# haosulab/ActiveZero

Hardware: AMD Instinct MI355X
Metric: stereo pairs/sec (540x960, D=192) fwd+bwd (higher is better)
Workload: dtype f32; 1 GPU; configs[1]: PSMNet 540x960 (padded to 544 rows) D=192 fwd+bwd+Adam, supervised disparity loss, batch 4 per GPU; global_batch=4, height=540, width=960, maxdisp=192, parallelism=dp1

## Files before the change

### activezero_amd/csrc/az_conv3d_c1.hip

```cpp
#include "az_common.h"
#include "az_launch_math.h"

#define C1_TH 8
#define C1_TW 32
#define C1_VS 36
#define C1_GP 36
typedef float c1_f2 __attribute__((ext_vector_type(2)));
#define C1_FMA2(a, b, c) __builtin_elementwise_fma(a, b, c)


#define C1F_TH 8
#define C1F_TW 16
template <int CTRL>
__device__ __forceinline__ float c1_dpp_add(float v) {
    return v + __builtin_bit_cast(float, __builtin_amdgcn_update_dpp(0, __builtin_bit_cast(int, v), CTRL, 0xf, 0xf, true));
}
__global__ void __launch_bounds__(256)
c1_fwd_kernel(float *__restrict__ out, const float *__restrict__ in, const float *__restrict__ w,
              const float *__restrict__ addend, const float *__restrict__ in_scale,
              const float *__restrict__ in_shift, int D, int H, int W, int tiles_x, int dseg) {
    constexpr int SX = C1F_TW + 2, SY = C1F_TH + 2;
    __shared__ __attribute__((aligned(16))) float slab[SY * SX * C1_VS];
    const int tx0 = (blockIdx.x % tiles_x) * C1F_TW, ty0 = (blockIdx.x / tiles_x) * C1F_TH;
    const int d0 = blockIdx.y * dseg, d1 = min(d0 + dseg, D), b = blockIdx.z;
    const int cp = threadIdx.x & 15, grp = threadIdx.x >> 4;
    const int ly = grp >> 1, lx0 = (grp & 1) * 8;
    const int oh = ty0 + ly;
    c1_f2 wp[27];
#pragma unroll
    for (int t = 0; t < 27; ++t) wp[t] = c1_f2{w[(cp * 2 + 0) * 27 + t], w[(cp * 2 + 1) * 27 + t]};
    c1_f2 a_prev[8], a_cur[8], a_next[8];
#pragma unroll
    for (int j = 0; j < 8; ++j) { a_prev[j] = c1_f2{0.f, 0.f}; a_cur[j] = c1_f2{0.f, 0.f}; a_next[j] = c1_f2{0.f, 0.f}; }
    constexpr int NQ = SY * SX * 8, NLD = (NQ + 255) / 256;
    float4 pre[NLD];
    const bool affine = in_scale != nullptr;
    float4 isc = make_float4(1.f, 1.f, 1.f, 1.f), ish = make_float4(0.f, 0.f, 0.f, 0.f);
    if (affine) {
        isc = reinterpret_cast<const float4 *>(in_scale)[threadIdx.x & 7];
        ish = reinterpret_cast<const float4 *>(in_shift)[threadIdx.x & 7];
    }
    unsigned okbits = 0;
    auto issue = [&](int id) {
        okbits = 0;
#pragma unroll
        for (int it = 0; it < NLD; ++it) {
            const int q = threadIdx.x + 256 * it, v = q >> 3, part = q & 7;
            const int sy = v / SX, sx = v - sy * SX;
            const int ih = ty0 - 1 + sy, iw = tx0 - 1 + sx;
            pre[it] = make_float4(0.f, 0.f, 0.f, 0.f);
            if (q < NQ && id >= 0 && id < D && ih >= 0 && ih < H && iw >= 0 && iw < W) {
                pre[it] = *reinterpret_cast<const float4 *>(
                    in + ((((size_t)b * D + id) * H + ih) * W + iw) * 32 + part * 4);
                okbits |= 1u << it;
            }
        }
    };
    issue(d0 - 1);
    for (int id = d0 - 1; id <= d1; ++id) {
        if (id >= 0 && id < D) {
            __syncthreads();
#pragma unroll
            for (int it = 0; it < NLD; ++it) {
                const int q = threadIdx.x + 256 * it;
                float4 v = pre[it];
                if (affine && ((okbits >> it) & 1u)) {
                    v.x = az_relu(fmaf(v.x, isc.x, ish.x)); v.y = az_relu(fmaf(v.y, isc.y, ish.y));
                    v.z = az_relu(fmaf(v.z, isc.z, ish.z)); v.w = az_relu(fmaf(v.w, isc.w, ish.w));
                }
                if (q < NQ) *reinterpret_cast<float4 *>(&slab[(q >> 3) * C1_VS + (q & 7) * 4]) = v;
            }
            __syncthreads();
        }
        if (id < d1) issue(id + 1);
        if (id >= 0 && id < D) {
#pragma unroll
            for (int kh = 0; kh < 3; ++kh) {
                c1_f2 r[10];
                const float *row = &slab[((ly + kh) * SX + lx0) * C1_VS + cp * 2];
#pragma unroll
                for (int i = 0; i < 10; ++i) {
                    const float2 x = *reinterpret_cast<const float2 *>(row + i * C1_VS);
                    r[i] = c1_f2{x.x, x.y};
                }
#pragma unroll
                for (int kw = 0; kw < 3; ++kw)
#pragma unroll
                    for (int j = 0; j < 8; ++j) {
                        a_next[j] = C1_FMA2(r[j + kw], wp[kh * 3 + kw], a_next[j]);
                        a_cur[j] = C1_FMA2(r[j + kw], wp[9 + kh * 3 + kw], a_cur[j]);
                        a_prev[j] = C1_FMA2(r[j + kw], wp[18 + kh * 3 + kw], a_prev[j]);
                    }
            }
        }
        const int od = id - 1;
        if (od >= d0 && od < d1) {
            float mine = 0.f;
#pragma unroll
            for (int j = 0; j < 8; ++j) {
                float v = a_prev[j][0] + a_prev[j][1];
                v = c1_dpp_add<0xB1>(v);
                v = c1_dpp_add<0x4E>(v);
                v = c1_dpp_add<0x141>(v);
                v = c1_dpp_add<0x140>(v);
                mine = (cp == j) ? v : mine;
            }
            const int ow = tx0 + lx0 + cp;
            if (cp < 8 && oh < H && ow < W) {
                const size_t o = (((size_t)b * D + od) * H + oh) * W + ow;
                out[o] = addend ? mine + addend[o] : mine;
            }
        }
#pragma unroll
        for (int j = 0; j < 8; ++j) { a_prev[j] = a_cur[j]; a_cur[j] = a_next[j]; a_next[j] = c1_f2{0.f, 0.f}; }
    }
}

__device__ __forceinline__ void c1_load_gtile(float *gt, const float *__restrict__ gout, int b,
                                              int od, int ty0, int tx0, int D, int H, int W) {
    constexpr int SX = C1_TW + 2, SY = C1_TH + 2;
    for (int q = threadIdx.x; q < 3 * SY * SX; q += 256) {
        const int sx = q % SX;
        const int r = q / SX;
        const int sy = r % SY, sd = r / SY;
        const int gd = od - 1 + sd, gh = ty0 - 1 + sy, gw = tx0 - 1 + sx;
        gt[r * C1_GP + sx] = (gd >= 0 && gd < D && gh >= 0 && gh < H && gw >= 0 && gw < W)
                                 ? gout[(((size_t)b * D + gd) * H + gh) * W + gw] : 0.f;
    }
}
__device__ __forceinline__ void c1_row6(float (&r)[6], const float *gt, int pd, int sy, int lx0) {
    const float *row = static_cast<const float *>(__builtin_assume_aligned(gt + (pd * (C1_TH + 2) + sy) * C1_GP + lx0, 16));
    const float4 a = *reinterpret_cast<const float4 *>(row);
    const float2 c = *reinterpret_cast<const float2 *>(row + 4);
    r[0] = a.x; r[1] = a.y; r[2] = a.z; r[3] = a.w; r[4] = c.x; r[5] = c.y;
}

__global__ void __launch_bounds__(256)
c1_dgrad_kernel(float *__restrict__ gin, const float *__restrict__ gout,
                const float *__restrict__ w, int D, int H, int W, int tiles_x) {
    constexpr int SY = C1_TH + 2;
    __shared__ __attribute__((aligned(16))) float gt[3 * SY * C1_GP];
    const int tx0 = (blockIdx.x % tiles_x) * C1_TW, ty0 = (blockIdx.x / tiles_x) * C1_TH;
    const int od = blockIdx.y, b = blockIdx.z;
    c1_load_gtile(gt, gout, b, od, ty0, tx0, D, H, W);
    const int cp = threadIdx.x & 15, grp = threadIdx.x >> 4;
    c1_f2 wp[27];
#pragma unroll
    for (int t = 0; t < 27; ++t) wp[t] = c1_f2{w[(cp * 2 + 0) * 27 + t], w[(cp * 2 + 1) * 27 + t]};
    __syncthreads();
#pragma unroll 1
    for (int p = 0; p < C1_TH * C1_TW / 128; ++p) {
        const int gi = p * 16 + grp, ly = gi >> 2, lx0 = (gi & 3) * 8;
        const int oh = ty0 + ly;
        c1_f2 acc[8];
#pragma unroll
        for (int j = 0; j < 8; ++j) acc[j] = c1_f2{0.f, 0.f};
#pragma unroll
        for (int kd = 0; kd < 3; ++kd)
#pragma unroll
            for (int kh = 0; kh < 3; ++kh) {
                float r[12];
                {
                    const float *row = static_cast<const float *>(__builtin_assume_aligned(
                        gt + ((2 - kd) * SY + ly + 2 - kh) * C1_GP + lx0, 16));
                    const float4 a = *reinterpret_cast<const float4 *>(row);
                    const float4 c = *reinterpret_cast<const float4 *>(row + 4);
                    const float2 e = *reinterpret_cast<const float2 *>(row + 8);
                    r[0] = a.x; r[1] = a.y; r[2] = a.z; r[3] = a.w; r[4] = c.x; r[5] = c.y; r[6] = c.z; r[7] = c.w;
                    r[8] = e.x; r[9] = e.y;
                }
#pragma unroll
                for (int kw = 0; kw < 3; ++kw) {
                    const int t = (kd * 3 + kh) * 3 + kw;
#pragma unroll
                    for (int j = 0; j < 8; ++j) {
                        const c1_f2 g2 = {r[j + 2 - kw], r[j + 2 - kw]};
                        acc[j] = C1_FMA2(g2, wp[t], acc[j]);
                    }
                }
            }
#pragma unroll
        for (int j = 0; j < 8; ++j) asm volatile("" : "+v"(acc[j]));
        if (oh < H) {
            float *dst = gin + ((((size_t)b * D + od) * H + oh) * W + tx0 + lx0) * 32 + cp * 2;
#pragma unroll
            for (int j = 0; j < 8; ++j)
                if (tx0 + lx0 + j < W) *reinterpret_cast<float2 *>(dst + j * 32) = make_float2(acc[j][0], acc[j][1]);
        }
    }
}

__global__ void __launch_bounds__(256)
c1_wgrad_kernel(float *__restrict__ gw, const float *__restrict__ in,
                const float *__restrict__ gout, const float *__restrict__ in_scale,
                const float *__restrict__ in_shift, int D, int H, int W, int tiles_x, int tiles_y,
                long long ntiles) {
    constexpr int SY = C1_TH + 2;
    __shared__ __attribute__((aligned(16))) float gt[3 * SY * C1_GP];
    __shared__ float red[864];
    for (int q = threadIdx.x; q < 864; q += 256) red[q] = 0.f;
    const int quad = threadIdx.x & 7, grp = threadIdx.x >> 3;
    const bool affine = in_scale != nullptr;
    float4 isc = make_float4(1.f, 1.f, 1.f, 1.f), ish = make_float4(0.f, 0.f, 0.f, 0.f);
    if (affine) {
        isc = reinterpret_cast<const float4 *>(in_scale)[quad];
        ish = reinterpret_cast<const float4 *>(in_shift)[quad];
    }
    c1_f2 a01[27], a23[27];
#pragma unroll
    for (int t = 0; t < 27; ++t) { a01[t] = c1_f2{0.f, 0.f}; a23[t] = c1_f2{0.f, 0.f}; }
    for (long long item = blockIdx.x; item < ntiles; item += gridDim.x) {
        long long r = item;
        const int tx0 = (int)(r % tiles_x) * C1_TW; r /= tiles_x;
        const int ty0 = (int)(r % tiles_y) * C1_TH; r /= tiles_y;
        const int od = (int)(r % D);
        const int b = (int)(r / D);
        __syncthreads();
        c1_load_gtile(gt, gout, b, od, ty0, tx0, D, H, W);
        __syncthreads();
#pragma unroll 1
        for (int p = 0; p < C1_TH * C1_TW / 128; ++p) {
            const int gi = p * 32 + grp, ly = gi >> 3, lx0 = (gi & 7) * 4;
            const int ih = ty0 + ly;
            c1_f2 x01[4], x23[4];
            const float *src = in + ((((size_t)b * D + od) * H + ih) * W + tx0 + lx0) * 32 + quad * 4;
#pragma unroll
            for (int j = 0; j < 4; ++j) {
                float4 x = make_float4(0.f, 0.f, 0.f, 0.f);
                if (ih < H && tx0 + lx0 + j < W) {
                    x = *reinterpret_cast<const float4 *>(src + j * 32);
                    if (affine) {
                        x.x = az_relu(fmaf(x.x, isc.x, ish.x)); x.y = az_relu(fmaf(x.y, isc.y, ish.y));
                        x.z = az_relu(fmaf(x.z, isc.z, ish.z)); x.w = az_relu(fmaf(x.w, isc.w, ish.w));
                    }
                }
                x01[j] = c1_f2{x.x, x.y}; x23[j] = c1_f2{x.z, x.w};
            }
#pragma unroll
            for (int kd = 0; kd < 3; ++kd)
#pragma unroll
                for (int kh = 0; kh < 3; ++kh) {
                    float r[6];
                    c1_row6(r, gt, 2 - kd, ly + 2 - kh, lx0);
#pragma unroll
                    for (int kw = 0; kw < 3; ++kw) {
                        const int t = (kd * 3 + kh) * 3 + kw;
#pragma unroll
                        for (int j = 0; j < 4; ++j) {
                            const c1_f2 g2 = {r[j + 2 - kw], r[j + 2 - kw]};
                            a01[t] = C1_FMA2(g2, x01[j], a01[t]);
                            a23[t] = C1_FMA2(g2, x23[j], a23[t]);
                        }
                    }
                }
        }
    }
#pragma unroll
    for (int c = 0; c < 4; ++c)
#pragma unroll
        for (int t = 0; t < 27; ++t) {
            float v = (c < 2 ? a01[t] : a23[t])[c & 1];
            v += __shfl_xor(v, 8); v += __shfl_xor(v, 16); v += __shfl_xor(v, 32);
            if ((threadIdx.x & 63) < 8) atomicAdd(&red[(quad * 4 + c) * 27 + t], v);
        }
    __syncthreads();
    for (int q = threadIdx.x; q < 864; q += 256) atomicAdd(&gw[q], red[q]);
}

static int c1_check(int B, int D, int H, int W) {
    if (!(B > 0 && D > 0 && H > 0 && W > 0)) return AZ_EINVAL;
    if (B > 65535 || D > 65535) return AZ_EUNSUPPORTED;
    return AZ_OK;
}

extern "C" int az_conv3d_c1_fwd(float *logits, const float *in, const float *w,
                                const float *addend, const float *in_scale, const float *in_shift, int B, int D,
                                int H, int W, void *stream) {
    AZ_REQUIRE_PTR(logits); AZ_REQUIRE_PTR(in); AZ_REQUIRE_PTR(w);
    if ((in_scale == nullptr) != (in_shift == nullptr)) return AZ_EINVAL;
    if (int e = c1_check(B, D, H, W)) return e;
    const int tiles_x = (W + C1F_TW - 1) / C1F_TW, tiles_y = (H + C1F_TH - 1) / C1F_TH;
    const int best = az_c1_fwd_dseg((long long)tiles_x * tiles_y * B, D);
    hipLaunchKernelGGL(c1_fwd_kernel, dim3(tiles_x * tiles_y, (D + best - 1) / best, B), dim3(256), 0,
                       az_stream(stream), logits, in, w, addend, in_scale, in_shift, D, H, W, tiles_x, best);
    return az_launch_status();
}

extern "C" int az_conv3d_c1_dgrad(float *grad_in, const float *grad_logits, const float *w,
                                  int B, int D, int H, int W, void *stream) {
    AZ_REQUIRE_PTR(grad_in); AZ_REQUIRE_PTR(grad_logits); AZ_REQUIRE_PTR(w);
    if (int e = c1_check(B, D, H, W)) return e;
    const int tiles_x = (W + C1_TW - 1) / C1_TW, tiles_y = (H + C1_TH - 1) / C1_TH;
    hipLaunchKernelGGL(c1_dgrad_kernel, dim3(tiles_x * tiles_y, D, B), dim3(256), 0,
                       az_stream(stream), grad_in, grad_logits, w, D, H, W, tiles_x);
    return az_launch_status();
}

extern "C" int az_conv3d_c1_wgrad(float *grad_w, const float *in, const float *grad_logits,
                                  const float *in_scale, const float *in_shift, int B, int D, int H, int W,
                                  void *stream) {
    AZ_REQUIRE_PTR(grad_w); AZ_REQUIRE_PTR(in); AZ_REQUIRE_PTR(grad_logits);
    if ((in_scale == nullptr) != (in_shift == nullptr)) return AZ_EINVAL;
    if (int e = c1_check(B, D, H, W)) return e;
    if (hipMemsetAsync(grad_w, 0, 864 * sizeof(float), az_stream(stream)) != hipSuccess)
        return AZ_ELAUNCH;
    const int tiles_x = (W + C1_TW - 1) / C1_TW, tiles_y = (H + C1_TH - 1) / C1_TH;
    const long long ntiles = az_c1_wgrad_tiles(B, D, H, W);
    const unsigned grid = (unsigned)az_c1_wgrad_grid(ntiles);
    hipLaunchKernelGGL(c1_wgrad_kernel, dim3(grid), dim3(256), 0, az_stream(stream), grad_w, in,
                       grad_logits, in_scale, in_shift, D, H, W, tiles_x, tiles_y, ntiles);
    return az_launch_status();
}

extern "C" int az_conv3d_c1_plan(long long *plan, int B, int D, int H, int W) {
    AZ_REQUIRE_PTR(plan);
    if (int e = c1_check(B, D, H, W)) return e;
    const long long patches = (long long)((W + C1F_TW - 1) / C1F_TW) * ((H + C1F_TH - 1) / C1F_TH) * B;
    const int dseg = az_c1_fwd_dseg(patches, D);
    const long long ntiles = az_c1_wgrad_tiles(B, D, H, W);
    plan[0] = dseg;
    plan[1] = patches * ((D + dseg - 1) / dseg);
    plan[2] = ntiles;
    plan[3] = az_c1_wgrad_grid(ntiles);
    return AZ_OK;
}
```

### activezero_amd/csrc/az_launch_math.h

```cpp
#pragma once
#if defined(__HIPCC__)
#define AZ_HD __host__ __device__ __forceinline__
#else
#define AZ_HD inline
#endif

AZ_HD int az_xcd_map(int bid, int nblk) {
    const int xcd = bid & 7, q8 = nblk >> 3, r8 = nblk & 7;
    return (xcd < r8 ? xcd * (q8 + 1) : r8 * (q8 + 1) + (xcd - r8) * q8) + (bid >> 3);
}

AZ_HD void az_conv_tile_decode(int lin, int map_mode, int band_rows, int tiles_x, int rows_y, int Dt, int &tix, int &tiy,
                               int &td, int &b) {
    tix = lin % tiles_x; lin /= tiles_x;
    if (map_mode >= 2) {
        const int per_b = Dt * rows_y;
        b = lin / per_b;
        int l = lin - b * per_b;
        const int full = (rows_y / band_rows) * band_rows * Dt;
        int band, rows;
        if (l < full) { band = l / (band_rows * Dt); l -= band * band_rows * Dt; rows = band_rows; }
        else { band = rows_y / band_rows; l -= full; rows = rows_y - band * band_rows; }
        td = l / rows;
        tiy = band * band_rows + (l - td * rows);
    } else {
        tiy = lin % rows_y; lin /= rows_y;
        td = lin % Dt;
        b = lin / Dt;
    }
}

#define AZ_S24_VS 24
AZ_HD int az_s24_write_off(int sy, int sx, int j, int pitch) {
    return (sy * pitch + sx) * AZ_S24_VS + ((j >> 1) ^ (sy & 1)) * 4 + (j & 1) * 2;
}
AZ_HD int az_s24_read_base(int rty, int rtx, int half, int parity, int pitch) {
    return (rty * pitch + rtx) * AZ_S24_VS + (half ^ ((rty + parity) & 1)) * 4;
}

inline void az_roll_segments(long long patches, int Do, int forced, int &nseg, int &seg_len) {
    if (forced > 0) {
        seg_len = forced < Do ? forced : Do;
        nseg = (Do + seg_len - 1) / seg_len;
        return;
    }
    long long best = -1;
    nseg = 1; seg_len = Do;
    for (int n = 1; n <= Do; ++n) {
        const int len = (Do + n - 1) / n;
        const int nn = (Do + len - 1) / len;
        if (nn != n) continue;
        const long long rounds = (patches * n + 511) / 512;
        const long long cost = rounds * (len + 2) * 3 + 2;
        if (best < 0 || cost < best) { best = cost; nseg = n; seg_len = len; }
    }
}

inline void az_t2roll_segments(long long patches, int Di, int &nseg, int &seg_len) {
    long long best = -1;
    nseg = 1; seg_len = Di;
    for (int n = 1; n <= Di; ++n) {
        const int len = (Di + n - 1) / n;
        if ((Di + len - 1) / len != n) continue;
        const long long rounds = (patches * n + 255) / 256;
        const long long cost = rounds * (len * 4 + 2) + 1;
        if (best < 0 || cost < best) { best = cost; nseg = n; seg_len = len; }
    }
}

inline void az_s2roll_segments(long long patches, int Do, int forced, int &nseg, int &seg_len, int slots = 512) {
    if (forced > 0) {
        seg_len = forced < Do ? forced : Do;
        nseg = (Do + seg_len - 1) / seg_len;
        return;
    }
    long long best = -1;
    nseg = 1; seg_len = Do;
    for (int n = 1; n <= Do; ++n) {
        const int len = (Do + n - 1) / n;
        if ((Do + len - 1) / len != n) continue;
        const long long rounds = (patches * n + slots - 1) / slots;
        const long long cost = rounds * (27LL * len + 4 * (2 * len + 1) + 4);
        if (best < 0 || cost < best) { best = cost; nseg = n; seg_len = len; }
    }
}

inline void az_c2r_segments(long long patches, int N, int &nseg, int &seg_len) {
    long long best = -1;
    nseg = 1; seg_len = N;
    for (int n = 1; n <= N; ++n) {
        const int len = (N + n - 1) / n;
        if ((N + len - 1) / len != n) continue;
        const long long rounds = (patches * n + 511) / 512;
        const long long cost = rounds * (len * 3 + 2);
        if (best < 0 || cost < best) { best = cost; nseg = n; seg_len = len; }
    }
}

#define AZ_C1_FWD_SLOTS 768
inline long long az_c1_fwd_cost(long long patches, int D, int dseg) {
    const long long blocks = patches * ((D + dseg - 1) / dseg);
    return ((blocks + AZ_C1_FWD_SLOTS - 1) / AZ_C1_FWD_SLOTS) * (dseg + 2);
}
inline int az_c1_fwd_dseg(long long patches, int D) {
    int best = 1;
    long long best_cost = -1;
    for (int nseg = 1; nseg <= D; ++nseg) {
        const int dseg = (D + nseg - 1) / nseg;
        const long long cost = az_c1_fwd_cost(patches, D, dseg);
        if (best_cost < 0 || cost < best_cost) { best_cost = cost; best = dseg; }
    }
    return best;
}
#define AZ_C1_WGRAD_MAX_GRID 2048
inline long long az_c1_wgrad_tiles(int B, int D, int H, int W) {
    return (long long)B * D * ((H + 7) / 8) * ((W + 31) / 32);
}
inline int az_c1_wgrad_grid(long long ntiles) {
    return (int)(ntiles < AZ_C1_WGRAD_MAX_GRID ? ntiles : AZ_C1_WGRAD_MAX_GRID);
}

AZ_HD void az_roll_decode(int lin, int tiles_x, int tyb, int nseg, int &tix, int &tiy, int &seg, int &b) {
    tix = lin % tiles_x; lin /= tiles_x;
    tiy = lin % tyb; lin /= tyb;
    seg = lin % nseg;
    b = lin / nseg;
}

#define AZ_R_SY 10
#define AZ_R_SX 18
#define AZ_R_NQ (AZ_R_SY * AZ_R_SX * 8)
AZ_HD bool az_roll_piece(int tid, int it, int &sy, int &sx) {
    const int vox = (tid >> 3) + 32 * it;
    sy = vox / AZ_R_SX;
    sx = vox - sy * AZ_R_SX;
    return tid + 256 * it < AZ_R_NQ;
}

inline int az_wgrad16_workgroups(long long ncols, int slots, int ntiles, int cap) {
    int best = 1;
    double best_score = -1.0;
    const int step = 8 / (ntiles > 2 ? 4 : ntiles);
    for (int w = slots; w >= slots / 4 && w >= 1; w -= step) {
        if (w > ncols) continue;
        const long long per = (ncols + w - 1) / w;
        const double score = (double)ncols / (double)(per * slots);
        if (score > best_score + 1e-9) { best_score = score; best = w; }
    }
    if (ncols < slots / 4) best = (int)(ncols > 0 ? ncols : 1);
    if (cap > 0 && cap < best) best = cap;
    return best;
}

AZ_HD int az_mfma32_c_row_h(int half, int reg) { return (reg & 3) + 8 * (reg >> 2) + 4 * half; }
AZ_HD int az_mfma32_c_row(int lane, int reg) { return az_mfma32_c_row_h(lane >> 5, reg); }
AZ_HD int az_mfma32_c_col(int lane) { return lane & 31; }
AZ_HD int az_mfma16_c_row(int lane, int reg) { return 4 * (lane >> 4) + reg; }
AZ_HD int az_mfma16_c_col(int lane) { return lane & 15; }

#define AZ_W16_ROWB 64
AZ_HD unsigned az_w16_half_swap(unsigned row) { return ((row >> 3) & 1u) << 5; }
AZ_HD int az_w16_piece_off(int row, int q) { return row * AZ_W16_ROWB + (((q & 7) * 8) ^ (((row >> 3) & 1) << 5)); }
AZ_HD unsigned az_w16_read_off(int lane, unsigned row0, unsigned ch0) {
    const unsigned row = row0 + ((unsigned)(lane & 15) >> 2);
    return row * AZ_W16_ROWB + (((ch0 + 4 * (unsigned)(lane & 3)) * 2) ^ az_w16_half_swap(row));
}
struct AzW16Lanes { unsigned a_lane, b_off[3][2]; int rp; };
AZ_HD AzW16Lanes az_w16_lanes(int lane, unsigned a_ch0, unsigned b_ch0) {
    const unsigned oct = (unsigned)lane >> 4;
    AzW16Lanes g;
    g.a_lane = az_w16_read_off(lane, 8 * oct, a_ch0);
    g.rp = (int)(oct >> 1);
    for (int kw = 0; kw < 3; ++kw)
        for (int h2 = 0; h2 < 2; ++h2) g.b_off[kw][h2] = az_w16_read_off(lane, 8 * (oct & 1) + kw + 4 * h2, b_ch0);
    return g;
}

struct AzC2w16Plan { int seg_rows, nrseg, wgs; long long ncols; };
inline AzC2w16Plan az_c2w16_plan(int B, int H, int W, int slots) {
    const int nwchunk = (W + 15) / 16;
    AzC2w16Plan p{};
    p.nrseg = 1; p.wgs = 1;
    double best = -1.0;
    for (int nseg = 1; nseg <= 16; ++nseg) {
        int rows = (H + nseg - 1) / nseg;
        rows += rows & 1;
        const int segs = (H + rows - 1) / rows;
        const long long cols = (long long)B * nwchunk * segs;
        const int w = (int)(cols < slots ? cols : slots);
        const long long per = (cols + w - 1) / w;
        const double balance = (double)cols / (double)(per * w);
        const double occ = (double)w / (double)slots;
        const double amort = (double)rows / (double)(rows + 4);
        const double score = balance * (0.5 + 0.5 * occ) * amort;
        if (score > best) { best = score; p.nrseg = segs; p.wgs = w; p.seg_rows = rows; }
    }
    p.ncols = (long long)B * nwchunk * p.nrseg;
    return p;
}

struct AzC2wPlan { int blocks_per_combo, hseg_rows, nhseg; long long nitems; };
inline AzC2wPlan az_c2w_plan(int B, int H, int W, int mt, int nt, int ncombo, int ring_rows) {
    const int nwchunk = (W + 15) / 16;
    const int slots = 256 * 8 / (mt * nt);
    const int wq = (slots / ncombo) & ~7;
    const int wmax = wq > 8 ? wq : 8;
    const int wmin = wmax / 2 > 8 ? wmax / 2 : 8;
    const long long base_items = (long long)B * nwchunk;
    double best = -1.0;
    int best_w = 8, best_rows = H;
    for (int nseg = 1; nseg <= (H < 32 ? H : 32); ++nseg) {
        const int rows = (H + nseg - 1) / nseg;
        const int segs = (H + rows - 1) / rows;
        const long long items = base_items * segs;
        for (int w = wmax; w >= wmin; w -= 8) {
            const long long per = (items + w - 1) / w;
            const double balance = (double)items / (double)(per * w);
            const double occ = (double)w / (double)wmax;
            const double amort = (double)rows / (double)(rows + ring_rows - 1 + 2);
            const double score = balance * (0.5 + 0.5 * occ) * amort;
            if (score > best) { best = score; best_w = w; best_rows = rows; }
        }
    }
    AzC2wPlan p{};
    p.blocks_per_combo = best_w;
    p.hseg_rows = best_rows;
    p.nhseg = (H + best_rows - 1) / best_rows;
    p.nitems = base_items * p.nhseg;
    if (p.nitems < p.blocks_per_combo) p.blocks_per_combo = (int)((p.nitems + 7) & ~7LL);
    return p;
}

#define AZ_S2W_FPOS 17
#define AZ_S2W_FROWQ (AZ_S2W_FPOS * 8)
#define AZ_S2W_NFQ (3 * 8 * AZ_S2W_FROWQ)
#define AZ_S2W_RING 17
AZ_HD bool az_s2w_fine_piece(int f, int &pk, int &j, int &pp, int &lrow) {
    pk = f / (8 * AZ_S2W_FROWQ);
    const int g = f - pk * (8 * AZ_S2W_FROWQ);
    j = g / AZ_S2W_FROWQ;
    pp = (g - j * AZ_S2W_FROWQ) >> 3;
    lrow = (pp & 1) ? 9 + (pp >> 1) : (pp >> 1);
    return f < AZ_S2W_NFQ;
}
AZ_HD int az_s2w_tap_row(int kw) { return kw == 0 ? 0 : kw == 1 ? 9 : 1; }
AZ_HD int az_s2w_ring_slot(int fr) { return (fr + 1) % AZ_S2W_RING; }
AZ_HD void az_s2w_col_decode(long long col, int Dc, int nwchunk, int &cd, int &wc, int &b) {
    cd = (int)(col % Dc); col /= Dc;
    wc = (int)(col % nwchunk);
    b = (int)(col / nwchunk);
}

inline bool az_fits_buffer_offset(long long bytes) { return bytes > 0 && bytes < 0xffffff00LL; }
```

Baseline: 47.54 pairs/s.

## March c1 conv3d backward kernels along depth with a rolling LDS plane ring

```diff
diff --git a/activezero_amd/csrc/az_conv3d_c1.hip b/activezero_amd/csrc/az_conv3d_c1.hip
--- a/activezero_amd/csrc/az_conv3d_c1.hip
+++ b/activezero_amd/csrc/az_conv3d_c1.hip
@@ -1,3 +1,5 @@
+#include <type_traits>
+
 #include "az_common.h"
 #include "az_launch_math.h"
 
@@ -116,20 +118,50 @@
     }
 }
 
-__device__ __forceinline__ void c1_load_gtile(float *gt, const float *__restrict__ gout, int b,
-                                              int od, int ty0, int tx0, int D, int H, int W) {
-    constexpr int SX = C1_TW + 2, SY = C1_TH + 2;
-    for (int q = threadIdx.x; q < 3 * SY * SX; q += 256) {
-        const int sx = q % SX;
-        const int r = q / SX;
-        const int sy = r % SY, sd = r / SY;
-        const int gd = od - 1 + sd, gh = ty0 - 1 + sy, gw = tx0 - 1 + sx;
-        gt[r * C1_GP + sx] = (gd >= 0 && gd < D && gh >= 0 && gh < H && gw >= 0 && gw < W)
-                                 ? gout[(((size_t)b * D + gd) * H + gh) * W + gw] : 0.f;
-    }
-}
-__device__ __forceinline__ void c1_row6(float (&r)[6], const float *gt, int pd, int sy, int lx0) {
-    const float *row = static_cast<const float *>(__builtin_assume_aligned(gt + (pd * (C1_TH + 2) + sy) * C1_GP + lx0, 16));
+#define C1_RING 4
+#define C1_PLANE ((C1_TH + 2) * C1_GP)
+struct c1_gstager {
+    long long idx[2];
+    int lds[2];
+    bool ok[2];
+    float v[2];
+    unsigned m[2];
+    int gd;
+    __device__ __forceinline__ void init(int b, int gd0, int ty0, int tx0, int D, int H, int W) {
+        constexpr int SX = C1_TW + 2, SY = C1_TH + 2;
+        gd = gd0;
+        const int gdc = min(max(gd0, 0), D - 1);
+#pragma unroll
+        for (int e = 0; e < 2; ++e) {
+            const int q = threadIdx.x + 256 * e, sy = q / SX, sx = q - sy * SX;
+            const int gh = ty0 - 1 + sy, gw = tx0 - 1 + sx;
+            lds[e] = q < SY * SX ? sy * C1_GP + sx : C1_TW + 2;
+            ok[e] = q < SY * SX && gh >= 0 && gh < H && gw >= 0 && gw < W;
+            idx[e] = (((long long)b * D + gdc) * H + min(max(gh, 0), H - 1)) * W + min(max(gw, 0), W - 1);
+            v[e] = 0.f;
+            m[e] = 0u;
+        }
+    }
+    __device__ __forceinline__ void fetch(const float *__restrict__ gout, int D, long long hw) {
+        const bool in = gd >= 0 && gd < D;
+        const long long step = (gd >= 0 && gd + 1 < D) ? hw : 0;
+#pragma unroll
+        for (int e = 0; e < 2; ++e) {
+            v[e] = gout[idx[e]];
+            m[e] = (in && ok[e]) ? ~0u : 0u;
+            idx[e] += step;
+        }
+        ++gd;
+    }
+    __device__ __forceinline__ void store(float *slot) const {
+#pragma unroll
+        for (int e = 0; e < 2; ++e)
+            slot[lds[e]] = __uint_as_float(__float_as_uint(v[e]) & m[e]);
+    }
+};
+__device__ __forceinline__ int c1_slot(int gd) { return (gd + 1) & (C1_RING - 1); }
+__device__ __forceinline__ void c1_row6(float (&r)[6], const float *p) {
+    const float *row = static_cast<const float *>(__builtin_assume_aligned(p, 16));
     const float4 a = *reinterpret_cast<const float4 *>(row);
     const float2 c = *reinterpret_cast<const float2 *>(row + 4);
     r[0] = a.x; r[1] = a.y; r[2] = a.z; r[3] = a.w; r[4] = c.x; r[5] = c.y;
@@ -137,124 +169,188 @@
 
 __global__ void __launch_bounds__(256)
 c1_dgrad_kernel(float *__restrict__ gin, const float *__restrict__ gout,
-                const float *__restrict__ w, int D, int H, int W, int tiles_x) {
-    constexpr int SY = C1_TH + 2;
-    __shared__ __attribute__((aligned(16))) float gt[3 * SY * C1_GP];
+                const float *__restrict__ w, int D, int H, int W, int tiles_x, int dseg) {
+    __shared__ __attribute__((aligned(16))) float ring[C1_RING * C1_PLANE];
     const int tx0 = (blockIdx.x % tiles_x) * C1_TW, ty0 = (blockIdx.x / tiles_x) * C1_TH;
-    const int od = blockIdx.y, b = blockIdx.z;
-    c1_load_gtile(gt, gout, b, od, ty0, tx0, D, H, W);
-    const int cp = threadIdx.x & 15, grp = threadIdx.x >> 4;
-    c1_f2 wp[27];
-#pragma unroll
-    for (int t = 0; t < 27; ++t) wp[t] = c1_f2{w[(cp * 2 + 0) * 27 + t], w[(cp * 2 + 1) * 27 + t]};
-    __syncthreads();
-#pragma unroll 1
-    for (int p = 0; p < C1_TH * C1_TW / 128; ++p) {
-        const int gi = p * 16 + grp, ly = gi >> 2, lx0 = (gi & 3) * 8;
-        const int oh = ty0 + ly;
-        c1_f2 acc[8];
-#pragma unroll
-        for (int j = 0; j < 8; ++j) acc[j] = c1_f2{0.f, 0.f};
-#pragma unroll
-        for (int kd = 0; kd < 3; ++kd)
-#pragma unroll
-            for (int kh = 0; kh < 3; ++kh) {
-                float r[12];
-                {
-                    const float *row = static_cast<const float *>(__builtin_assume_aligned(
-                        gt + ((2 - kd) * SY + ly + 2 - kh) * C1_GP + lx0, 16));
-                    const float4 a = *reinterpret_cast<const float4 *>(row);
-                    const float4 c = *reinterpret_cast<const float4 *>(row + 4);
-                    const float2 e = *reinterpret_cast<const float2 *>(row + 8);
-                    r[0] = a.x; r[1] = a.y; r[2] = a.z; r[3] = a.w; r[4] = c.x; r[5] = c.y; r[6] = c.z; r[7] = c.w;
-                    r[8] = e.x; r[9] = e.y;
-                }
-#pragma unroll
-                for (int kw = 0; kw < 3; ++kw) {
-                    const int t = (kd * 3 + kh) * 3 + kw;
-#pragma unroll
-                    for (int j = 0; j < 8; ++j) {
-                        const c1_f2 g2 = {r[j + 2 - kw], r[j + 2 - kw]};
-                        acc[j] = C1_FMA2(g2, wp[t], acc[j]);
-                    }
-                }
-            }
-#pragma unroll
-        for (int j = 0; j < 8; ++j) asm volatile("" : "+v"(acc[j]));
-        if (oh < H) {
-            float *dst = gin + ((((size_t)b * D + od) * H + oh) * W + tx0 + lx0) * 32 + cp * 2;
-#pragma unroll
-            for (int j = 0; j < 8; ++j)
-                if (tx0 + lx0 + j < W) *reinterpret_cast<float2 *>(dst + j * 32) = make_float2(acc[j][0], acc[j][1]);
-        }
-    }
-}
-
-__global__ void __launch_bounds__(256)
-c1_wgrad_kernel(float *__restrict__ gw, const float *__restrict__ in,
-                const float *__restrict__ gout, const float *__restrict__ in_scale,
-                const float *__restrict__ in_shift, int D, int H, int W, int tiles_x, int tiles_y,
-                long long ntiles) {
-    constexpr int SY = C1_TH + 2;
-    __shared__ __attribute__((aligned(16))) float gt[3 * SY * C1_GP];
-    __shared__ float red[864];
-    for (int q = threadIdx.x; q < 864; q += 256) red[q] = 0.f;
+    const int d0 = blockIdx.y * dseg, d1 = min(d0 + dseg, D), b = blockIdx.z;
     const int quad = threadIdx.x & 7, grp = threadIdx.x >> 3;
-    const bool affine = in_scale != nullptr;
-    float4 isc = make_float4(1.f, 1.f, 1.f, 1.f), ish = make_float4(0.f, 0.f, 0.f, 0.f);
-    if (affine) {
-        isc = reinterpret_cast<const float4 *>(in_scale)[quad];
-        ish = reinterpret_cast<const float4 *>(in_shift)[quad];
-    }
-    c1_f2 a01[27], a23[27];
-#pragma unroll
-    for (int t = 0; t < 27; ++t) { a01[t] = c1_f2{0.f, 0.f}; a23[t] = c1_f2{0.f, 0.f}; }
-    for (long long item = blockIdx.x; item < ntiles; item += gridDim.x) {
-        long long r = item;
-        const int tx0 = (int)(r % tiles_x) * C1_TW; r /= tiles_x;
-        const int ty0 = (int)(r % tiles_y) * C1_TH; r /= tiles_y;
-        const int od = (int)(r % D);
-        const int b = (int)(r / D);
+    const int lyl = grp >> 3, lx0 = (grp & 7) * 4;
+    const long long hw = (long long)H * W;
+    c1_gstager st;
+    st.init(b, d0 - 1, ty0, tx0, D, H, W);
+    st.fetch(gout, D, hw); st.store(ring + c1_slot(d0 - 1) * C1_PLANE);
+    st.fetch(gout, D, hw); st.store(ring + c1_slot(d0) * C1_PLANE);
+    st.fetch(gout, D, hw); st.store(ring + c1_slot(d0 + 1) * C1_PLANE);
+    c1_f2 w01[27], w23[27];
+#pragma unroll
+    for (int t = 0; t < 27; ++t) {
+        w01[t] = c1_f2{w[(quad * 4 + 0) * 27 + t], w[(quad * 4 + 1) * 27 + t]};
+        w23[t] = c1_f2{w[(quad * 4 + 2) * 27 + t], w[(quad * 4 + 3) * 27 + t]};
+    }
+    unsigned wok = 0;
+#pragma unroll
+    for (int j = 0; j < 4; ++j) wok |= (tx0 + lx0 + j < W ? 1u : 0u) << j;
+    long long go = ((((long long)b * D + d0) * H + ty0 + lyl) * W + tx0 + lx0) * 32 + quad * 4;
+    const int lane = lyl * C1_GP + lx0;
+    const bool full = ty0 + C1_TH <= H && tx0 + C1_TW <= W;
+    auto march = [&](auto fullc) {
+    constexpr bool FULL = decltype(fullc)::value;
+    for (int d = d0; d < d1; ++d, go += hw * 32) {
         __syncthreads();
-        c1_load_gtile(gt, gout, b, od, ty0, tx0, D, H, W);
-        __syncthreads();
-#pragma unroll 1
-        for (int p = 0; p < C1_TH * C1_TW / 128; ++p) {
-            const int gi = p * 32 + grp, ly = gi >> 3, lx0 = (gi & 7) * 4;
-            const int ih = ty0 + ly;
-            c1_f2 x01[4], x23[4];
-            const float *src = in + ((((size_t)b * D + od) * H + ih) * W + tx0 + lx0) * 32 + quad * 4;
-#pragma unroll
-            for (int j = 0; j < 4; ++j) {
-                float4 x = make_float4(0.f, 0.f, 0.f, 0.f);
-                if (ih < H && tx0 + lx0 + j < W) {
-                    x = *reinterpret_cast<const float4 *>(src + j * 32);
-                    if (affine) {
-                        x.x = az_relu(fmaf(x.x, isc.x, ish.x)); x.y = az_relu(fmaf(x.y, isc.y, ish.y));
-                        x.z = az_relu(fmaf(x.z, isc.z, ish.z)); x.w = az_relu(fmaf(x.w, isc.w, ish.w));
-                    }
-                }
-                x01[j] = c1_f2{x.x, x.y}; x23[j] = c1_f2{x.z, x.w};
-            }
+        st.fetch(gout, D, hw);
+        const float *gk[3] = {ring + c1_slot(d + 1) * C1_PLANE + lane, ring + c1_slot(d) * C1_PLANE + lane,
+                              ring + c1_slot(d - 1) * C1_PLANE + lane};
+#pragma unroll
+        for (int p = 0; p < C1_TH / 4; ++p) {
+            __builtin_amdgcn_sched_barrier(0);
+            c1_f2 a01[4], a23[4];
+#pragma unroll
+            for (int j = 0; j < 4; ++j) { a01[j] = c1_f2{0.f, 0.f}; a23[j] = c1_f2{0.f, 0.f}; }
 #pragma unroll
             for (int kd = 0; kd < 3; ++kd)
 #pragma unroll
                 for (int kh = 0; kh < 3; ++kh) {
                     float r[6];
-                    c1_row6(r, gt, 2 - kd, ly + 2 - kh, lx0);
+                    c1_row6(r, gk[kd] + (p * 4 + 2 - kh) * C1_GP);
 #pragma unroll
                     for (int kw = 0; kw < 3; ++kw) {
                         const int t = (kd * 3 + kh) * 3 + kw;
 #pragma unroll
                         for (int j = 0; j < 4; ++j) {
                             const c1_f2 g2 = {r[j + 2 - kw], r[j + 2 - kw]};
-                            a01[t] = C1_FMA2(g2, x01[j], a01[t]);
-                            a23[t] = C1_FMA2(g2, x23[j], a23[t]);
+                            a01[j] = C1_FMA2(g2, w01[t], a01[j]);
+                            a23[j] = C1_FMA2(g2, w23[t], a23[j]);
                         }
                     }
                 }
-        }
-    }
+#pragma unroll
+            for (int j = 0; j < 4; ++j) asm volatile("" : "+v"(a01[j]), "+v"(a23[j]));
+            float *dst = gin + go + (long long)p * 4 * W * 32;
+            if (FULL) {
+#pragma unroll
+                for (int j = 0; j < 4; ++j)
+                    *reinterpret_cast<float4 *>(dst + j * 32) = make_float4(a01[j][0], a01[j][1], a23[j][0], a23[j][1]);
+            } else if (ty0 + p * 4 + lyl < H) {
+#pragma unroll
+                for (int j = 0; j < 4; ++j)
+                    if ((wok >> j) & 1u)
+                        *reinterpret_cast<float4 *>(dst + j * 32) = make_float4(a01[j][0], a01[j][1], a23[j][0], a23[j][1]);
+            }
+        }
+        st.store(ring + c1_slot(d + 2) * C1_PLANE);
+    }
+    };
+    if (full) march(std::true_type{}); else march(std::false_type{});
+}
+
+__device__ __forceinline__ void c1_wgrad_pass(c1_f2 (&a01)[27], c1_f2 (&a23)[27], const float4 (&x)[4],
+                                              const float *const (&gk)[3], int p) {
+    c1_f2 x01[4], x23[4];
+#pragma unroll
+    for (int j = 0; j < 4; ++j) { x01[j] = c1_f2{x[j].x, x[j].y}; x23[j] = c1_f2{x[j].z, x[j].w}; }
+#pragma unroll
+    for (int kd = 0; kd < 3; ++kd)
+#pragma unroll
+        for (int kh = 0; kh < 3; ++kh) {
+            float r[6];
+            c1_row6(r, gk[kd] + (p * 4 + 2 - kh) * C1_GP);
+#pragma unroll
+            for (int kw = 0; kw < 3; ++kw) {
+                const int t = (kd * 3 + kh) * 3 + kw;
+#pragma unroll
+                for (int j = 0; j < 4; ++j) {
+                    const c1_f2 g2 = {r[j + 2 - kw], r[j + 2 - kw]};
+                    a01[t] = C1_FMA2(g2, x01[j], a01[t]);
+                    a23[t] = C1_FMA2(g2, x23[j], a23[t]);
+                }
+            }
+        }
+}
+
+template <bool AFFINE>
+__global__ void __launch_bounds__(256, 2)
+c1_wgrad_kernel(float *__restrict__ gw, const float *__restrict__ in,
+                const float *__restrict__ gout, const float *__restrict__ in_scale,
+                const float *__restrict__ in_shift, int D, int H, int W, int tiles_x, int dseg) {
+    __shared__ __attribute__((aligned(16))) float ring[C1_RING * C1_PLANE];
+    __shared__ float red[864];
+    for (int q = threadIdx.x; q < 864; q += 256) red[q] = 0.f;
+    const int tx0 = (blockIdx.x % tiles_x) * C1_TW, ty0 = (blockIdx.x / tiles_x) * C1_TH;
+    const int d0 = blockIdx.y * dseg, d1 = min(d0 + dseg, D), b = blockIdx.z;
+    const int quad = threadIdx.x & 7, grp = threadIdx.x >> 3;
+    const int lyl = grp >> 3, lx0 = (grp & 7) * 4;
+    const long long hw = (long long)H * W;
+    c1_gstager st;
+    st.init(b, d0 - 1, ty0, tx0, D, H, W);
+    st.fetch(gout, D, hw); st.store(ring + c1_slot(d0 - 1) * C1_PLANE);
+    st.fetch(gout, D, hw); st.store(ring + c1_slot(d0) * C1_PLANE);
+    st.fetch(gout, D, hw);
+    float4 isc = make_float4(1.f, 1.f, 1.f, 1.f), ish = make_float4(0.f, 0.f, 0.f, 0.f);
+    if (AFFINE) {
+        isc = reinterpret_cast<const float4 *>(in_scale)[quad];
+        ish = reinterpret_cast<const float4 *>(in_shift)[quad];
+    }
+    c1_f2 a01[27], a23[27];
+#pragma unroll
+    for (int t = 0; t < 27; ++t) { a01[t] = c1_f2{0.f, 0.f}; a23[t] = c1_f2{0.f, 0.f}; }
+    static_assert(C1_TH / 4 == 2, "the pass pipeline below is written for two passes per plane");
+    long long xi[2];
+    int xo[4];
+    unsigned okbits = 0;
+    {
+        const int x0 = min(tx0 + lx0, W - 1);
+#pragma unroll
+        for (int j = 0; j < 4; ++j) xo[j] = (min(tx0 + lx0 + j, W - 1) - x0) * 32;
+#pragma unroll
+        for (int p = 0; p < 2; ++p) {
+            const int ih = ty0 + p * 4 + lyl;
+            xi[p] = ((((long long)b * D + d0) * H + min(ih, H - 1)) * W + x0) * 32 + quad * 4;
+#pragma unroll
+            for (int j = 0; j < 4; ++j) okbits |= (ih < H && tx0 + lx0 + j < W ? 1u : 0u) << (p * 4 + j);
+        }
+    }
+    const int lane = lyl * C1_GP + lx0;
+    const bool full = ty0 + C1_TH <= H && tx0 + C1_TW <= W;
+    const long long idle = ((((long long)b * D + d0) * H + ty0) * W + tx0) * 32;
+    auto load = [&](float4 (&x)[4], int p, bool live) {
+#pragma unroll
+        for (int j = 0; j < 4; ++j) x[j] = *reinterpret_cast<const float4 *>(in + (live ? xi[p] + xo[j] : idle));
+        xi[p] += hw * 32;
+    };
+    auto prep = [&](float4 (&x)[4], int p) {
+#pragma unroll
+        for (int j = 0; j < 4; ++j) {
+            float4 v = x[j];
+            if (AFFINE) {
+                v.x = az_relu(fmaf(v.x, isc.x, ish.x)); v.y = az_relu(fmaf(v.y, isc.y, ish.y));
+                v.z = az_relu(fmaf(v.z, isc.z, ish.z)); v.w = az_relu(fmaf(v.w, isc.w, ish.w));
+            }
+            if (!full) {
+                const unsigned m = 0u - ((okbits >> (p * 4 + j)) & 1u);
+                v.x = __uint_as_float(__float_as_uint(v.x) & m); v.y = __uint_as_float(__float_as_uint(v.y) & m);
+                v.z = __uint_as_float(__float_as_uint(v.z) & m); v.w = __uint_as_float(__float_as_uint(v.w) & m);
+            }
+            x[j] = v;
+        }
+    };
+    float4 xa[4], xb[4];
+    load(xa, 0, true);
+    auto plane = [&](int d) {
+        st.store(ring + c1_slot(d + 1) * C1_PLANE);
+        __syncthreads();
+        st.fetch(gout, D, hw);
+        const float *const gk[3] = {ring + c1_slot(d + 1) * C1_PLANE + lane, ring + c1_slot(d) * C1_PLANE + lane,
+                                    ring + c1_slot(d - 1) * C1_PLANE + lane};
+        load(xb, 1, true);
+        __builtin_amdgcn_sched_barrier(0);
+        prep(xa, 0); c1_wgrad_pass(a01, a23, xa, gk, 0);
+        __builtin_amdgcn_sched_barrier(0);
+        load(xa, 0, d + 1 < d1);
+        __builtin_amdgcn_sched_barrier(0);
+        prep(xb, 1); c1_wgrad_pass(a01, a23, xb, gk, 1);
+        __builtin_amdgcn_sched_barrier(0);
+    };
+    for (int d = d0; d < d1; ++d) plane(d);
 #pragma unroll
     for (int c = 0; c < 4; ++c)
 #pragma unroll
@@ -291,8 +387,9 @@
     AZ_REQUIRE_PTR(grad_in); AZ_REQUIRE_PTR(grad_logits); AZ_REQUIRE_PTR(w);
     if (int e = c1_check(B, D, H, W)) return e;
     const int tiles_x = (W + C1_TW - 1) / C1_TW, tiles_y = (H + C1_TH - 1) / C1_TH;
-    hipLaunchKernelGGL(c1_dgrad_kernel, dim3(tiles_x * tiles_y, D, B), dim3(256), 0,
-                       az_stream(stream), grad_in, grad_logits, w, D, H, W, tiles_x);
+    const int dseg = az_c1_bwd_dseg((long long)tiles_x * tiles_y * B, D);
+    hipLaunchKernelGGL(c1_dgrad_kernel, dim3(tiles_x * tiles_y, (D + dseg - 1) / dseg, B), dim3(256), 0,
+                       az_stream(stream), grad_in, grad_logits, w, D, H, W, tiles_x, dseg);
     return az_launch_status();
 }
 
@@ -305,10 +402,14 @@
     if (hipMemsetAsync(grad_w, 0, 864 * sizeof(float), az_stream(stream)) != hipSuccess)
         return AZ_ELAUNCH;
     const int tiles_x = (W + C1_TW - 1) / C1_TW, tiles_y = (H + C1_TH - 1) / C1_TH;
-    const long long ntiles = az_c1_wgrad_tiles(B, D, H, W);
-    const unsigned grid = (unsigned)az_c1_wgrad_grid(ntiles);
-    hipLaunchKernelGGL(c1_wgrad_kernel, dim3(grid), dim3(256), 0, az_stream(stream), grad_w, in,
-                       grad_logits, in_scale, in_shift, D, H, W, tiles_x, tiles_y, ntiles);
+    const int dseg = az_c1_bwd_dseg((long long)tiles_x * tiles_y * B, D);
+    const dim3 grid(tiles_x * tiles_y, (D + dseg - 1) / dseg, B);
+    if (in_scale != nullptr)
+        hipLaunchKernelGGL(c1_wgrad_kernel<true>, grid, dim3(256), 0, az_stream(stream), grad_w, in, grad_logits,
+                           in_scale, in_shift, D, H, W, tiles_x, dseg);
+    else
+        hipLaunchKernelGGL(c1_wgrad_kernel<false>, grid, dim3(256), 0, az_stream(stream), grad_w, in, grad_logits,
+                           in_scale, in_shift, D, H, W, tiles_x, dseg);
     return az_launch_status();
 }
 
diff --git a/activezero_amd/csrc/az_launch_math.h b/activezero_amd/csrc/az_launch_math.h
--- a/activezero_amd/csrc/az_launch_math.h
+++ b/activezero_amd/csrc/az_launch_math.h
@@ -118,6 +118,18 @@
 }
 inline int az_c1_wgrad_grid(long long ntiles) {
     return (int)(ntiles < AZ_C1_WGRAD_MAX_GRID ? ntiles : AZ_C1_WGRAD_MAX_GRID);
+}
+#define AZ_C1_BWD_SLOTS 512
+inline int az_c1_bwd_dseg(long long columns, int D) {
+    int best = 1;
+    long long best_cost = -1;
+    for (int nseg = 1; nseg <= D; ++nseg) {
+        const int dseg = (D + nseg - 1) / nseg;
+        const long long blocks = columns * ((D + dseg - 1) / dseg);
+        const long long cost = ((blocks + AZ_C1_BWD_SLOTS - 1) / AZ_C1_BWD_SLOTS) * (dseg + 1);
+        if (best_cost < 0 || cost < best_cost) { best_cost = cost; best = dseg; }
+    }
+    return best;
 }
 
 AZ_HD void az_roll_decode(int lin, int tiles_x, int tyb, int nseg, int &tix, int &tiy, int &seg, int &b) {
```

Result: no change. 47.95 pairs/s, median of 6 (+0.9%).
